# samiwilf/torchrec-oldfork

Hardware: AMD Instinct MI355X
Metric: samples/sec Criteo-1TB DLRM batch 65536 (higher is better)
Workload: dtype f32; 1 GPU; DLRM Criteo-1TB shape: 26 tables (177.9M rows, 84.85 GiB fp32, D=128), 13 dense, pooling factor 1, dense 512-256-128, over 1024-1024-512-256-1, fused exact SGD; global_batch=65536, local_batch=65536, parallelism=mp1: 26 table-wise + 0 row-wise + 0 replicated (data-parallel) tables, dense dp1, ids=uniform, distinct_batches=32, seed=0, data_ranks=1

## Files before the change

include/tbe_hip.h:

```cpp
#ifndef TBE_HIP_H_
#define TBE_HIP_H_

#include <stddef.h>
#include <stdint.h>

#ifdef __cplusplus
extern "C" {
#endif

#define TBE_OK 0
#define TBE_ERR_INVALID_ARGUMENT (-1)
#define TBE_ERR_LAUNCH (-2)
#define TBE_ERR_WORKSPACE (-3)
#define TBE_ERR_UNSUPPORTED (-4)

#define TBE_POOL_SUM 0
#define TBE_POOL_MEAN 1
#define TBE_POOL_NONE 2

#define TBE_OPT_EXACT_SGD 0
#define TBE_OPT_EXACT_ROWWISE_ADAGRAD 1
#define TBE_OPT_ADAM 2
#define TBE_OPT_EXACT_ADAGRAD 3
#define TBE_OPT_DENSE_GRAD 100
// ... 120 lines not shown
int tbe_block_bucketize(const void* lengths, int32_t len_elem_size, int64_t lengths_size,
                        const void* indices, int32_t idx_elem_size, int64_t N,
                        const void* block_sizes, int32_t F, int32_t my_size,
                        const float* weights, int32_t bucketize_pos, int32_t sequence,
                        void* new_lengths, void* new_indices, float* new_weights,
                        void* new_pos, void* unbucketize_permute, void* workspace,
                        size_t workspace_bytes, void* stream);

int tbe_a2a_pooled_unpack(const float* recv, float* out, const int32_t* dim_sum_per_rank,
                          int32_t W, int32_t B_local, int32_t D_total,
                          int32_t dims_multiple_of_4, float scale, void* stream);
int tbe_a2a_pooled_pack(const float* grad, float* send, const int32_t* dim_sum_per_rank,
                        int32_t W, int32_t B_local, int32_t D_total,
                        int32_t dims_multiple_of_4, float scale, void* stream);

int tbe_pooled_exchange_unpack(const float* recv, float* out, const int32_t* feat_out_col,
                               const int32_t* feat_src, const int32_t* feat_slab_col,
                               const int64_t* slab_offset, const int32_t* slab_stride,
                               int32_t Fg, int32_t W, int32_t B_local, int32_t D_total,
                               int32_t all_multiple_of_4, float scale, void* stream);
int tbe_pooled_exchange_pack(const float* grad, float* send, const int32_t* feat_out_col,
                             const int32_t* feat_src, const int32_t* feat_slab_col,
                             const int64_t* slab_offset, const int32_t* slab_stride,
                             int32_t Fg, int32_t W, int32_t B_local, int32_t D_total,
                             int32_t all_multiple_of_4, float scale, void* stream);

int tbe_dlrm_interaction_forward_f32(const float* dense, const float* sparse, int32_t B,
                                     int32_t F, int32_t D, float* out, int64_t out_row_stride,
                                     void* stream);
int tbe_dlrm_interaction_backward_f32(const float* dense, const float* sparse,
                                      const float* grad_out, int64_t grad_row_stride, int32_t B, int32_t F, int32_t D,
                                      float* grad_dense, float* grad_sparse, void* stream);

size_t tbe_relu_backward_bias_grad_workspace_bytes(int64_t B, int32_t N);
int tbe_relu_backward_bias_grad_f32(const float* grad_out, const float* act, int64_t B, int32_t N,
                                    float* grad_in, float* bias_grad, void* workspace,
                                    size_t workspace_bytes, void* stream);

size_t tbe_weighted_colsum_workspace_bytes(int64_t B, int32_t N);
int tbe_weighted_colsum_f32(const float* x, const float* w, int64_t B, int32_t N, float* out,
                            void* workspace, size_t workspace_bytes, void* stream);

int64_t tbe_colsum_row_blocks(int64_t B, int32_t N);
int tbe_relu_backward_bias_partials_f32(const float* grad_out, const float* act, int64_t B, int32_t N,
                                        float* grad_in, float* partial, size_t partial_bytes, void* stream);
int tbe_weighted_colsum_partials_f32(const float* x, const float* w, int64_t B, int32_t N, float* partial,
                                     size_t partial_bytes, void* stream);

int tbe_multi_chunk_sum_f32(const int64_t* seg_table, int32_t nseg, int64_t max_numel, float* dst, float scale,
                            void* stream);
int tbe_multi_chunk_sum_host_table_f32(const int64_t* host_seg_table, int32_t nseg, int64_t max_numel, float* dst,
                                       float scale, void* stream);

size_t tbe_bce_with_logits_workspace_bytes(void);
int tbe_bce_with_logits_f32(const float* logits, const void* labels, int32_t label_elem_size, int64_t B, float* loss,
                            float* dlogits, void* workspace, size_t workspace_bytes, void* stream);

int tbe_jagged_2d_to_dense_f32(const float* values, const int64_t* offsets, int32_t B,
                               int32_t D, int32_t max_L, float* dense, void* stream);

int tbe_dense_to_jagged_2d_f32(const float* dense, const int64_t* offsets, int32_t B, int32_t D,
                               int32_t max_L, int64_t N, float* values, void* stream);

int tbe_offsets_range(const int64_t* offsets, int64_t n, int64_t range_size, int64_t* out,
                      void* stream);

// ... 8 lines not shown
```

torchrec-oldfork_amd/csrc/dlrm_interaction.hip:

```cpp
#include <algorithm>
#include <cstdlib>

#include "common.hpp"

namespace tbe {

using f32x4 = __attribute__((ext_vector_type(4))) float;

__device__ __forceinline__ void wave_lds_fence() { __builtin_amdgcn_wave_barrier(); }

__device__ __forceinline__ int triu_index(int i, int j, int R) { return i * (2 * R - i - 1) / 2 + (j - i - 1); }

__device__ __forceinline__ int triu_row(int p, int R) {
  const int t = 2 * R - 1;
  int i = static_cast<int>((static_cast<float>(t) - sqrtf(static_cast<float>(t * t - 8 * p))) * 0.5f);
  i = max(0, min(i, R - 2));
  while (i + 1 <= R - 2 && (i + 1) * (2 * R - (i + 1) - 1) / 2 <= p) ++i;
  while (i > 0 && i * (2 * R - i - 1) / 2 > p) --i;
  return i;
}

template <int D>
struct XLoader {
  static constexpr int LOG_V = (D == 16 ? 2 : D == 32 ? 3 : D == 64 ? 4 : D == 128 ? 5 : 6);
// ... 365 lines not shown
    wave_lds_fence();
#pragma unroll
    for (int m = 0; m < 2; ++m)
#pragma unroll
      for (int n = 0; n < NT; ++n)
#pragma unroll
        for (int q = 0; q < 4; ++q) {
          const int row = 16 * m + 4 * kq + q;
          if (row < R) xs[row * XS + 16 * n + r16] = acc[m][n][q];
        }
    wave_lds_fence();
#pragma unroll
    for (int i = 0; i < MAXV; ++i) {
      const int v = lane + i * kWave;
      if (v < nvec) {
        const int r = v >> LOG_V;
        const int c = (v & ((1 << LOG_V) - 1)) * 4;
        float4 x = ld4(xs + r * XS + c);
        if (r == 0) {
          x.x += gdense.x;
          x.y += gdense.y;
          x.z += gdense.z;
          x.w += gdense.w;
          st4(grad_dense + static_cast<int64_t>(b) * D + c, x);
        } else {
          st4(grad_sparse + (static_cast<int64_t>(b) * F + (r - 1)) * D + c, x);
        }
      }
    }
    wave_lds_fence();
  }
}

}

using namespace tbe;

static unsigned interaction_grid(int B) {
  const int64_t want = (static_cast<int64_t>(B) + 3) / 4;
  return static_cast<unsigned>(std::max<int64_t>(1, std::min<int64_t>(want, 256 * 2)));
}

template <typename K>
static bool reserve_lds(K kernel, size_t bytes) {
  return hipFuncSetAttribute(reinterpret_cast<const void*>(kernel), hipFuncAttributeMaxDynamicSharedMemorySize,
                             static_cast<int>(bytes)) == hipSuccess;
}

extern "C" int tbe_dlrm_interaction_forward_f32(const float* dense, const float* sparse, int32_t B, int32_t F,
                                                int32_t D, float* out, int64_t out_row_stride, void* stream) {
  TBE_REQUIRE(B >= 0 && F >= 1 && F <= 31, "tbe_dlrm_interaction_forward_f32: F=%d outside [1, 31]", F);
  TBE_REQUIRE(out_row_stride >= D + (F + 1) * F / 2, "tbe_dlrm_interaction_forward_f32: out_row_stride %lld < D + F(F+1)/2",
              (long long)out_row_stride);
  TBE_REQUIRE(D == 16 || D == 32 || D == 64 || D == 128 || D == 256,
              "tbe_dlrm_interaction_forward_f32: D=%d not in {16,32,64,128,256}", D);
  if (B == 0) return TBE_OK;
  TBE_REQUIRE(dense && sparse && out, "tbe_dlrm_interaction_forward_f32: null pointer");
  TBE_REQUIRE(((reinterpret_cast<uintptr_t>(dense) | reinterpret_cast<uintptr_t>(sparse)) & 15) == 0,
              "tbe_dlrm_interaction_forward_f32: inputs must be 16-B aligned");
  const int R = F + 1, P = R * (R - 1) / 2;
  const size_t lds = 4 * static_cast<size_t>((P + 3) & ~3) * sizeof(float);
  hipStream_t st = static_cast<hipStream_t>(stream);
  const int64_t want = (static_cast<int64_t>(B) + 3) / 4;
  const dim3 grid(static_cast<unsigned>(std::max<int64_t>(1, std::min<int64_t>(want, 256 * (D <= 128 ? 4 : 2)))));
  if (D == 64 || D == 128) {
    const int rpi = 64 / (D / 4);
// ... 33 lines not shown
  TBE_REQUIRE(B >= 0 && F >= 1 && F <= 27, "tbe_dlrm_interaction_backward_f32: F=%d outside [1, 27]", F);
  TBE_REQUIRE(grad_row_stride >= D + (F + 1) * F / 2, "tbe_dlrm_interaction_backward_f32: grad_row_stride %lld < D + F(F+1)/2",
              (long long)grad_row_stride);
  TBE_REQUIRE(D == 16 || D == 32 || D == 64 || D == 128, "tbe_dlrm_interaction_backward_f32: D=%d not in {16,32,64,128}", D);
  if (B == 0) return TBE_OK;
  TBE_REQUIRE(dense && sparse && grad_out && grad_dense && grad_sparse, "tbe_dlrm_interaction_backward_f32: null pointer");
  TBE_REQUIRE(((reinterpret_cast<uintptr_t>(dense) | reinterpret_cast<uintptr_t>(sparse) |
                reinterpret_cast<uintptr_t>(grad_dense) | reinterpret_cast<uintptr_t>(grad_sparse)) & 15) == 0,
              "tbe_dlrm_interaction_backward_f32: tensors must be 16-B aligned");
  hipStream_t st = static_cast<hipStream_t>(stream);
  const size_t lds = 4 * (static_cast<size_t>(28) * (D + 16) + 32 * 34) * sizeof(float);
  const dim3 grid(interaction_grid(B));
  static bool attr_set = false;
  if (!attr_set) {
    const size_t big = 4 * (28 * (128 + 16) + 32 * 34) * sizeof(float);
    if (!reserve_lds(interaction_bwd_kernel<8>, big) || !reserve_lds(interaction_bwd_kernel<4>, big)) {
      set_error("tbe_dlrm_interaction_backward_f32: cannot reserve LDS");
      return TBE_ERR_LAUNCH;
    }
    attr_set = true;
  }
#define TBE_IB(NT) \
  hipLaunchKernelGGL(interaction_bwd_kernel<NT>, grid, dim3(256), lds, st, dense, sparse, grad_out, grad_dense, grad_sparse, B, F, grad_row_stride)
  switch (D) {
    case 16: TBE_IB(1); break;
    case 32: TBE_IB(2); break;
    case 64: TBE_IB(4); break;
    default: TBE_IB(8); break;
  }
#undef TBE_IB
  TBE_CHECK_LAUNCH("tbe_dlrm_interaction_backward_f32");
  return TBE_OK;
}
```

torchrec-oldfork_amd/fbgemm_gpu/_lib.py:

```python
import ctypes
import os
from typing import Optional

import torch

_HERE = os.path.dirname(os.path.abspath(__file__))
LIB_PATH = os.path.normpath(os.path.join(_HERE, "..", "lib", "libtbe_hip.so"))

c_void_p = ctypes.c_void_p
c_i32 = ctypes.c_int32
c_i64 = ctypes.c_int64
c_size = ctypes.c_size_t
c_float = ctypes.c_float


class OptimizerArgs(ctypes.Structure):

    _fields_ = [
        ("optimizer", c_i32),
        ("learning_rate", c_float),
        ("eps", c_float),
        ("weight_decay", c_float),
        ("beta1", c_float),
        ("beta2", c_float),
# ... 67 lines not shown
    "tbe_permute_2d_workspace_bytes": (c_size, [c_i32, c_i32, c_i32]),
    "tbe_permute_2d_lengths": (
        ctypes.c_int,
        [c_void_p, c_i32, c_i32, c_i32, c_void_p, c_i32, c_void_p, c_void_p, c_void_p, c_void_p,
         c_size, c_void_p],
    ),
    "tbe_permute_2d_data": (
        ctypes.c_int,
        [c_void_p, c_i32, c_i32, c_void_p, c_void_p, c_void_p, c_void_p, c_i32, c_void_p, c_void_p,
         c_i32, c_void_p],
    ),
    "tbe_bucketize_workspace_bytes": (c_size, [c_i64, c_i32]),
    "tbe_block_bucketize": (
        ctypes.c_int,
        [c_void_p, c_i32, c_i64, c_void_p, c_i32, c_i64, c_void_p, c_i32, c_i32, c_void_p, c_i32,
         c_i32, c_void_p, c_void_p, c_void_p, c_void_p, c_void_p, c_void_p, c_size, c_void_p],
    ),
    "tbe_a2a_pooled_unpack": (
        ctypes.c_int, [c_void_p, c_void_p, c_void_p, c_i32, c_i32, c_i32, c_i32, c_float, c_void_p]),
    "tbe_a2a_pooled_pack": (
        ctypes.c_int, [c_void_p, c_void_p, c_void_p, c_i32, c_i32, c_i32, c_i32, c_float, c_void_p]),
    "tbe_pooled_exchange_unpack": (
        ctypes.c_int,
        [c_void_p, c_void_p, c_void_p, c_void_p, c_void_p, c_void_p, c_void_p, c_i32, c_i32, c_i32,
         c_i32, c_i32, c_float, c_void_p]),
    "tbe_pooled_exchange_pack": (
        ctypes.c_int,
        [c_void_p, c_void_p, c_void_p, c_void_p, c_void_p, c_void_p, c_void_p, c_i32, c_i32, c_i32,
         c_i32, c_i32, c_float, c_void_p]),
    "tbe_dlrm_interaction_forward_f32": (
        ctypes.c_int, [c_void_p, c_void_p, c_i32, c_i32, c_i32, c_void_p, c_i64, c_void_p]),
    "tbe_dlrm_interaction_backward_f32": (
        ctypes.c_int, [c_void_p, c_void_p, c_void_p, c_i64, c_i32, c_i32, c_i32, c_void_p, c_void_p, c_void_p]),
    "tbe_relu_backward_bias_grad_workspace_bytes": (c_size, [c_i64, c_i32]),
    "tbe_relu_backward_bias_grad_f32": (
        ctypes.c_int, [c_void_p, c_void_p, c_i64, c_i32, c_void_p, c_void_p, c_void_p, c_size, c_void_p]),
    "tbe_weighted_colsum_workspace_bytes": (c_size, [c_i64, c_i32]),
    "tbe_weighted_colsum_f32": (
        ctypes.c_int, [c_void_p, c_void_p, c_i64, c_i32, c_void_p, c_void_p, c_size, c_void_p]),
    "tbe_colsum_row_blocks": (c_i64, [c_i64, c_i32]),
    "tbe_relu_backward_bias_partials_f32": (
        ctypes.c_int, [c_void_p, c_void_p, c_i64, c_i32, c_void_p, c_void_p, c_size, c_void_p]),
    "tbe_weighted_colsum_partials_f32": (
        ctypes.c_int, [c_void_p, c_void_p, c_i64, c_i32, c_void_p, c_size, c_void_p]),
    "tbe_multi_chunk_sum_f32": (ctypes.c_int, [c_void_p, c_i32, c_i64, c_void_p, c_float, c_void_p]),
    "tbe_multi_chunk_sum_host_table_f32": (ctypes.c_int, [c_void_p, c_i32, c_i64, c_void_p, c_float, c_void_p]),
    "tbe_bce_with_logits_workspace_bytes": (c_size, []),
    "tbe_bce_with_logits_f32": (
        ctypes.c_int, [c_void_p, c_void_p, c_i32, c_i64, c_void_p, c_void_p, c_void_p, c_size, c_void_p]),
    "tbe_jagged_2d_to_dense_f32": (
        ctypes.c_int, [c_void_p, c_void_p, c_i32, c_i32, c_i32, c_void_p, c_void_p]),
    "tbe_dense_to_jagged_2d_f32": (
        ctypes.c_int, [c_void_p, c_void_p, c_i32, c_i32, c_i32, c_i64, c_void_p, c_void_p]),
    "tbe_offsets_range": (ctypes.c_int, [c_void_p, c_i64, c_i64, c_void_p, c_void_p]),
    "tbe_copy_rows": (ctypes.c_int, [c_void_p, c_i64, c_void_p, c_i32, c_i64, c_void_p, c_void_p]),
}

_lib: Optional[ctypes.CDLL] = None


def load() -> ctypes.CDLL:
    global _lib
    if _lib is not None:
        return _lib
    if not os.path.exists(LIB_PATH):
        raise ImportError(
# ... 77 lines not shown
```

torchrec-oldfork_amd/fbgemm_gpu/split_table_batched_embeddings_ops.py:

```python
import enum
import os
import types
from ctypes import byref as ctypes_byref
from dataclasses import dataclass
from typing import List, Optional, Tuple

import torch
from torch import nn

from . import _lib, _streams
from ._lib import CacheDesc, OptimizerArgs, check, ptr, raise_on_faults, require_gpu, stream_ptr, workspace
from .split_embedding_configs import EmbOptimType as OptimType
from .split_embedding_configs import SparseType


_FLAG_WEIGHTED = 2


class EmbeddingLocation(enum.IntEnum):
    DEVICE = 0
    MANAGED = 1
    MANAGED_CACHING = 2
    HOST = 3

# ... 878 lines not shown
        prepare = torch.is_grad_enabled() and (
            mode in (True, "1") or (mode == "auto" and indices.numel() <= self.overlap_backward_sort_max_ids))
        out = _FusedLookup.apply(self.placeholder_autograd_tensor, self, indices, offsets,
                                 per_sample_weights, B, prepare)
        self._enforce_bounds_check_mode()
        return out

    def forward_into(self, out: torch.Tensor, out_offsets: torch.Tensor, row_stride: int, indices: torch.Tensor,
                     offsets: torch.Tensor, per_sample_weights: Optional[torch.Tensor] = None) -> torch.Tensor:
        indices, offsets, per_sample_weights, B = self._check_inputs(indices, offsets, per_sample_weights)
        if self._cache is not None:
            indices = self._cache.prefetch(self._real_layout(), indices, offsets, B, torch.is_grad_enabled())
        mode = self.overlap_backward_sort
        prepare = torch.is_grad_enabled() and (
            mode in (True, "1") or (mode == "auto" and indices.numel() <= self.overlap_backward_sort_max_ids))
        out = _FusedLookupInto.apply(out, self.placeholder_autograd_tensor, self, indices, offsets,
                                     per_sample_weights, B, out_offsets, int(row_stride), prepare)
        self._enforce_bounds_check_mode()
        return out

    def lookup_no_autograd(self, indices: torch.Tensor, offsets: torch.Tensor,
                           per_sample_weights: Optional[torch.Tensor] = None, into=None):
        indices, offsets, per_sample_weights, B = self._check_inputs(indices, offsets, per_sample_weights)
        if self._cache is not None:
            indices = self._cache.prefetch(self._real_layout(), indices, offsets, B, True)
        rec = LookupRecord(indices, offsets, per_sample_weights, B, (into[1], int(into[2])) if into is not None else None)
        out = self._forward_impl(indices, offsets, per_sample_weights, B, into=into)
        mode = self.overlap_backward_sort
        if mode in (True, "1") or (mode == "auto" and indices.numel() <= self.overlap_backward_sort_max_ids_explicit):
            rec.prepared = self._prepare_or_defer(rec, indices, offsets, B, per_sample_weights is not None)
        self._enforce_bounds_check_mode()
        return out, rec

    def backward_no_autograd(self, rec: "LookupRecord", grad_out: torch.Tensor) -> None:
        self.iter += 1
        self._backward_impl(grad_out, rec.indices, rec.offsets, rec.per_sample_weights, rec.B, self._optimizer_struct(),
                            prepared=rec.prepared, layout=rec.layout)
        rec.prepared = None
        if self._cache is not None:
            self._cache.after_backward()


class _DenseLookup(torch.autograd.Function):
    @staticmethod
    def forward(ctx, weights, module, indices, offsets, per_sample_weights, B):
        ctx.module = module
        ctx.B = B
        ctx.save_for_backward(indices, offsets, per_sample_weights)
        return module._forward_impl(indices, offsets, per_sample_weights, B)

    @staticmethod
    def backward(ctx, grad_out):
        indices, offsets, psw = ctx.saved_tensors
        module = ctx.module
        grad_w = torch.zeros_like(module.weights)
        state0 = module._dense_grad_ptrs(grad_w)
        opt = OptimizerArgs(_OPT_DENSE_GRAD, 0.0, 0.0, 0.0, 0.0, 0.0, 1)
        module._backward_impl(grad_out, indices, offsets, psw, ctx.B, opt, state0_override=state0,
                              state0_aligned=grad_w.data_ptr() % 16 == 0)
        return grad_w, None, None, None, None, None


class DenseTableBatchedEmbeddingBagsCodegen(_TBEBase):

    def __init__(
        self,
# ... 81 lines not shown
```

torchrec-oldfork_amd/torchrec_amd/distributed/embeddingbag.py:

```python
import os
from typing import Any, Callable, Dict, Iterator, List, Optional, Tuple

import torch
import torch.distributed as dist
from torch import nn

from ..modules.embedding_configs import EmbeddingBagConfig, pooling_type_to_pooling_mode
from ..modules.embedding_modules import EmbeddingBagCollection
from ..profiling import label
from ..sparse.jagged_tensor import KeyedJaggedTensor, KeyedTensor
from . import _device_ops
from .planner import rw_block_size, rw_shard_rows
from .types import Awaitable, LazyAwaitable, NoWait, ParameterSharding, ShardingEnv, ShardingType

GRADIENT_DIVISION = True
FORCE_EXCHANGE = os.environ.get("TORCHREC_AMD_FORCE_EXCHANGE", "0") == "1"


def set_gradient_division(val: bool) -> None:
    global GRADIENT_DIVISION
    GRADIENT_DIVISION = val


def _gather_rows(mat: torch.Tensor, order: List[int], order_dev: torch.Tensor) -> torch.Tensor:
# ... 900 lines not shown
            buf = self._output_buffer
            use_buf = buf is not None and buf.numel() == B * self._D_total
            if self._dp_module is None and not use_buf:
                emb = self._emb_module(dist_input.values, dist_input.offsets, dist_input.weights)
                return NoWait(KeyedTensor(keys, lpe, emb))
            out = (self._alias_output_buffer(B) if use_buf
                   else torch.empty((B, self._D_total), dtype=torch.float32, device=self._device))
            if self._emb_module is not None:
                out = self._emb_module.forward_into(out, self._sharded_out_off, self._D_total, dist_input.values,
                                                    dist_input.offsets, dist_input.weights)
            return NoWait(KeyedTensor(keys, lpe, self._dp_fill(out, dist_input)))
        if self._emb_module is not None:
            with label("## tbe_lookup ##"):
                emb = self._emb_module(dist_input.values, dist_input.offsets, dist_input.weights)
        else:
            emb = torch.zeros((self._world_size * B, 0), dtype=torch.float32, device=self._device,
                              requires_grad=True)
        state = _ExchangeState(self, B)
        recv = _ExchangeReq.apply(emb, state)
        return _OutputAwaitable(
            lambda: KeyedTensor(keys, lpe, self._dp_fill(_ExchangeWait.apply(recv, state), dist_input)))

    def explicit_step_supported(self, batch_size: int) -> bool:
        buf = self._output_buffer
        return (self._emb_module is not None and buf is not None
                and buf.numel() == batch_size * self._D_total and hasattr(self._emb_module, "lookup_no_autograd")
                and (self._dp_module is None or hasattr(self._dp_module, "lookup_no_autograd")))

    def compute_explicit(self, dist_input: SparseFeaturesDist, prefetched: bool = False) -> "ExplicitLookupStep":
        if not self.explicit_step_supported(dist_input.batch_size):
            raise RuntimeError("compute_explicit: not available for this configuration (explicit_step_supported())")
        return ExplicitLookupStep(self, dist_input, halves=self.half_batch_exchange, early_replicated_lookup=not prefetched)

    def forward(self, features: KeyedJaggedTensor) -> Awaitable[KeyedTensor]:
        return self.compute_and_output_dist(self.input_dist(features).wait())


class ExplicitLookupStep:

    def __init__(self, owner: "ShardedEmbeddingBagCollection", dist_input: SparseFeaturesDist, halves: bool = False,
                 early_replicated_lookup: bool = True) -> None:
        self.o, self.d = owner, dist_input
        self.halves = bool(halves and owner._exchange)
        self.epoch = owner._weights_epoch
        self.dp_rec = None
        self.state: Optional[_ExchangeState] = None
        self._grad: Optional[torch.Tensor] = None
        self._early_dp = False
        self._dp_sort_pending = False
        if owner._exchange:
            m = owner._emb_module
            can_defer = hasattr(m, "launch_deferred_backward_sort") and not getattr(m, "defer_backward_sort", False)
            if can_defer:
                m.defer_backward_sort = True
            try:
                with label("## tbe_lookup ##"):
                    emb, self.rec = m.lookup_no_autograd(dist_input.values, dist_input.offsets, dist_input.weights)
            finally:
                if can_defer:
                    m.defer_backward_sort = False
            self.state = _ExchangeState(owner, dist_input.batch_size)
            if self.halves:
                self.state.start_forward_halves(emb)
            else:
                self.state.start_forward(emb, allow_static=True)
            self._early_dp = owner._dp_module is not None and early_replicated_lookup
            if self._early_dp:
                v, offs, w = dist_input.dp
# ... 114 lines not shown
```

torchrec-oldfork_amd/torchrec_amd/distributed/train_pipeline.py:

```python
from typing import Any, Iterator, List, Optional, Tuple

import torch

from fbgemm_gpu._streams import side_stream

from ..profiling import label
from .model_parallel import DistributedModelParallel


class _PipelinedEBC:

    def __init__(self, sharded, pipeline: "TrainPipelineSparseDist") -> None:
        self.sharded = sharded
        self.pipeline = pipeline

    def _dist_input(self, features):
        req = self.pipeline._requests.pop(id(self.sharded), None)
        if req is None:
            return self.sharded.input_dist(features).wait()
        cur = torch.cuda.current_stream()
        with label("## wait_sparse_data_dist ##"):
            with torch.cuda.stream(self.pipeline._data_dist_stream):
                dist_in = req.wait()
            cur.wait_stream(self.pipeline._data_dist_stream)
        dist_in.record_stream(cur)
        return dist_in

    def forward(self, features):
        return self.sharded.compute_and_output_dist(self._dist_input(features))

    def compute_explicit(self, features, prefetched: bool = False):
        if not hasattr(self.sharded, "compute_explicit") or not self.sharded.explicit_step_supported(features.stride()):
            return None
        return self.sharded.compute_explicit(self._dist_input(features), prefetched=prefetched)


class TrainPipelineSparseDist:
    def __init__(self, model: torch.nn.Module, optimizer: Any, device: torch.device, hip_graphs: bool = False,
                 prefetch_lookup: Optional[bool] = None) -> None:
        self._model, self._optimizer, self._device = model, optimizer, device
        self._hip_graphs = hip_graphs and device.type == "cuda"
        if isinstance(model, DistributedModelParallel) and model.is_data_parallel_wrapped():
            self._hip_graphs = False
        use_streams = device.type == "cuda"
        self._memcpy_stream = side_stream(device) if use_streams else None
        self._data_dist_stream = side_stream(device) if use_streams else None
        self._requests = {}
        import os
        env = os.environ.get("TORCHREC_AMD_PREFETCH_LOOKUP")
        self._prefetch = bool(prefetch_lookup) if prefetch_lookup is not None else (env == "1" if env is not None else None)
        self._batch_i = None
        self._batch_ip1 = None
        self._batch_ip2 = None
        self._connected = False
        dmp = model if isinstance(model, DistributedModelParallel) else None
        self._sharded = dmp.sharded_modules() if dmp is not None else []
        self._install()

    def _install(self) -> None:
        self._wrappers: List[_PipelinedEBC] = []
        for s in self._sharded:
            w = getattr(s, "_pipelined", None)
            if w is None or w.pipeline is not self:
                w = _PipelinedEBC(s, self)
                s.forward = w.forward
                s._pipelined = w
            self._wrappers.append(w)
# ... 114 lines not shown
```

torchrec-oldfork_amd/torchrec_amd/models/dlrm.py:

```python
import os
from typing import Dict, List, Optional, Tuple

import torch
from torch import nn

from ..modules.mlp import MLP, LinearOut
from ..profiling import label
from ..sparse.jagged_tensor import KeyedJaggedTensor, KeyedTensor


class SparseArch(nn.Module):

    def __init__(self, embedding_bag_collection: nn.Module) -> None:
        super().__init__()
        self.embedding_bag_collection = embedding_bag_collection
        cfgs = embedding_bag_collection.embedding_bag_configs
        assert cfgs, "Embedding bag collection cannot be empty!"
        self.D: int = cfgs[0].embedding_dim
        self._sparse_feature_names: List[str] = [n for c in cfgs for n in c.feature_names]
        self.F: int = len(self._sparse_feature_names)

    def start(self, features: KeyedJaggedTensor):
        return self.embedding_bag_collection(features)

# ... 61 lines not shown
        buf = torch.empty((B, stride), dtype=torch.float32, device=dense.device)
        with torch.cuda.device(dense.device):
            check(_lib.load().tbe_dlrm_interaction_forward_f32(ptr(dense), ptr(sparse), B, F, D, ptr(buf), stride,
                                                               stream_ptr(dense.device)),
                  "tbe_dlrm_interaction_forward_f32")
        ctx.save_for_backward(dense, sparse)
        ctx.grad_sinks = grad_sinks
        return buf if stride == width else buf[:, :width]

    @staticmethod
    def backward(ctx, grad_out):
        from fbgemm_gpu import _lib
        from fbgemm_gpu._lib import check, ptr, stream_ptr

        dense, sparse = ctx.saved_tensors
        B, F, D = sparse.shape
        width = D + (F + 1) * F // 2
        if grad_out.shape != (B, width):
            raise RuntimeError(f"dot interaction backward: grad_out {tuple(grad_out.shape)} has the wrong shape")
        if grad_out.dtype != torch.float32 or grad_out.stride(1) != 1 or grad_out.stride(0) < width:
            grad_out = grad_out.float().contiguous()
        if ctx.grad_sinks is not None:
            gd, gs = ctx.grad_sinks
            if (gd.shape != dense.shape or gs.shape != sparse.shape or not gd.is_contiguous() or not gs.is_contiguous()
                    or gd.dtype != torch.float32 or gs.dtype != torch.float32 or gd.device != dense.device):
                raise RuntimeError("dot interaction backward: gradient sinks do not match the inputs")
        else:
            gd, gs = torch.empty_like(dense), torch.empty_like(sparse)
        with torch.cuda.device(dense.device):
            check(_lib.load().tbe_dlrm_interaction_backward_f32(ptr(dense), ptr(sparse), ptr(grad_out), grad_out.stride(0),
                                                                B, F, D, ptr(gd), ptr(gs), stream_ptr(dense.device)),
                  "tbe_dlrm_interaction_backward_f32")
        return gd, gs, None, None


def _fused_interaction_ok(dense: torch.Tensor, sparse: torch.Tensor) -> bool:
    F, D = sparse.shape[1], sparse.shape[2]
    return (dense.is_cuda and dense.dtype == torch.float32 and sparse.dtype == torch.float32
            and 1 <= F <= 27 and D in (16, 32, 64, 128))


class InteractionArch(nn.Module):

    def __init__(self, num_sparse_features: int) -> None:
        super().__init__()
        self.F = num_sparse_features
        self.fused = True
        self.pad_rows = os.environ.get("TORCHREC_AMD_PAD_INTERACTION", "0") == "1"
        self.grad_sinks = None
        self.register_buffer("triu_indices", torch.triu_indices(self.F + 1, self.F + 1, offset=1), persistent=False)

    def forward(self, dense_features: torch.Tensor, sparse_features: torch.Tensor) -> torch.Tensor:
        if self.F <= 0:
            return dense_features
        if self.fused and _fused_interaction_ok(dense_features, sparse_features):
            return _FusedDotInteraction.apply(dense_features, sparse_features, self.pad_rows, self.grad_sinks)
        combined = torch.cat((dense_features.unsqueeze(1), sparse_features), dim=1)
        interactions = torch.bmm(combined, combined.transpose(1, 2))
        flat = interactions[:, self.triu_indices[0], self.triu_indices[1]]
        return torch.cat((dense_features, flat), dim=1)


class OverArch(nn.Module):
    def __init__(self, in_features: int, layer_sizes: List[int], device: Optional[torch.device] = None) -> None:
        super().__init__()
        if len(layer_sizes) <= 1:
            raise ValueError("OverArch must have multiple layers.")
        self.model = nn.Sequential(
            MLP(in_features, layer_sizes[:-1], bias=True, activation="relu", device=device),
            LinearOut(layer_sizes[-2], layer_sizes[-1], bias=True, device=device))

    def forward(self, features: torch.Tensor) -> torch.Tensor:
        return self.model(features)


class DLRM(nn.Module):
    def __init__(self, embedding_bag_collection: nn.Module, dense_in_features: int,
                 dense_arch_layer_sizes: List[int], over_arch_layer_sizes: List[int],
                 dense_device: Optional[torch.device] = None) -> None:
        super().__init__()
        cfgs = embedding_bag_collection.embedding_bag_configs
        assert len(cfgs) > 0, "At least one embedding bag is required"
        D = cfgs[0].embedding_dim
        assert all(c.embedding_dim == D for c in cfgs), "All EmbeddingBagConfigs must have the same dimension"
        if dense_arch_layer_sizes[-1] != D:
            raise ValueError(f"embedding_bag_collection dimension ({D}) and final dense arch layer size "
                             f"({dense_arch_layer_sizes[-1]}) must match.")
        self.sparse_arch = SparseArch(embedding_bag_collection)
        F = self.sparse_arch.F
        self.dense_arch = DenseArch(dense_in_features, dense_arch_layer_sizes, device=dense_device)
        self.inter_arch = InteractionArch(F)
        over_in = D + (F + 1) * F // 2
        self.over_arch = OverArch(over_in, over_arch_layer_sizes, device=dense_device)
        if dense_device is not None:
            self.inter_arch.to(dense_device)

    def forward(self, dense_features: torch.Tensor, sparse_features: KeyedJaggedTensor) -> torch.Tensor:
        pending = self.sparse_arch.start(sparse_features)
        embedded_dense = self.dense_arch(dense_features)
        embedded_sparse = self.sparse_arch.finish(pending)
        concatenated = self.inter_arch(dense_features=embedded_dense, sparse_features=embedded_sparse)
        return self.over_arch(concatenated)




class _FusedBCEWithLogits(torch.autograd.Function):
    @staticmethod
    def forward(ctx, logits, labels):
        from ..distributed import _device_ops

        loss, dlogits = torch.ops.tbe_hip.bce_with_logits(logits, labels)
        ctx.save_for_backward(dlogits)
        return loss

    @staticmethod
    def backward(ctx, grad_out):
        (dlogits,) = ctx.saved_tensors
        return dlogits * grad_out, None


def bce_with_logits_mean(loss_fn: nn.Module, logits: torch.Tensor, labels: torch.Tensor) -> torch.Tensor:
    if (logits.is_cuda and logits.dtype == torch.float32 and logits.dim() == 1 and labels.shape == logits.shape
            and type(loss_fn) is nn.BCEWithLogitsLoss and loss_fn.reduction == "mean" and loss_fn.weight is None
            and loss_fn.pos_weight is None and logits.numel() > 0 and labels.dtype in (torch.float32, torch.int64)):
        return _FusedBCEWithLogits.apply(logits, labels)
    return loss_fn(logits, labels.float())


class _Head(nn.Module):
# ... 455 lines not shown
```

Measured before the change: 7.747 million samples/s.

## Fuse embedding row gather into DLRM interaction forward and backward kernels

Adds gather-interaction kernels that read embedding rows straight from the table weights by index (pooling factor 1), so the separate TBE pooled-output write and re-read is skipped. The forward uses LDS-DMA loads with software prefetch of the next sample's ids and rows. The backward re-gathers the rows to compute gradients and then calls the fused SGD backward directly. A deferred lookup path in the sharded EBC and DLRM forward turns this on when single-rank, table-wise, fixed-length-1 conditions hold. The cost is extra random row reads in backward and new code paths that only cover restricted configurations.

```diff
diff --git a/include/tbe_hip.h b/include/tbe_hip.h
--- a/include/tbe_hip.h
+++ b/include/tbe_hip.h
@@ -176,6 +176,15 @@
                                       const float* grad_out, int64_t grad_row_stride, int32_t B, int32_t F, int32_t D,
                                       float* grad_dense, float* grad_sparse, void* stream);
 
+int tbe_dlrm_interaction_gather_forward_f32(const float* dense, const uint64_t* feat_weights, const int64_t* feat_rows,
+                                            const int64_t* feat_window, const int64_t* indices, int32_t B, int32_t F,
+                                            int32_t D, float* out, int64_t out_row_stride, int32_t* bounds_errors,
+                                            void* stream);
+int tbe_dlrm_interaction_gather_backward_f32(const float* dense, const uint64_t* feat_weights, const int64_t* feat_rows,
+                                             const int64_t* feat_window, const int64_t* indices, const float* grad_out,
+                                             int64_t grad_row_stride, int32_t B, int32_t F, int32_t D, float* grad_dense,
+                                             float* grad_sparse, int32_t* bounds_errors, void* stream);
+
 size_t tbe_relu_backward_bias_grad_workspace_bytes(int64_t B, int32_t N);
 int tbe_relu_backward_bias_grad_f32(const float* grad_out, const float* act, int64_t B, int32_t N,
                                     float* grad_in, float* bias_grad, void* workspace,
diff --git a/torchrec-oldfork_amd/csrc/dlrm_interaction.hip b/torchrec-oldfork_amd/csrc/dlrm_interaction.hip
--- a/torchrec-oldfork_amd/csrc/dlrm_interaction.hip
+++ b/torchrec-oldfork_amd/csrc/dlrm_interaction.hip
@@ -421,6 +421,350 @@
   }
 }
 
+
+__device__ __attribute__((aligned(16))) float g_zero_row[256];
+
+struct GatherLane {
+  RowWindow win;
+  uint64_t base;
+  bool counts;
+};
+__device__ __forceinline__ GatherLane load_gather_lane(const uint64_t* feat_weights, const int64_t* feat_rows,
+                                                       const int64_t* feat_window, int lane, int F) {
+  GatherLane g;
+  const int f = min(lane, F - 1);
+  g.win = load_window(feat_rows, feat_window, f);
+  g.base = feat_weights[f];
+  g.counts = lane < F;
+  return g;
+}
+template <int D>
+__device__ __forceinline__ uint64_t gather_row_address(const GatherLane& g, int64_t id, uint64_t miss, int& nbad) {
+  int64_t local;
+  const int cls = classify_id(g.win, id, local);
+  if (cls == kIdBad && g.counts) ++nbad;
+  return cls == kIdLocal ? g.base + static_cast<uint64_t>(local) * (D * sizeof(float)) : miss;
+}
+__device__ __forceinline__ void report_bad_ids(int nbad, int32_t* bounds_errors) {
+  if (bounds_errors == nullptr) return;
+#pragma unroll
+  for (int o = 32; o > 0; o >>= 1) nbad += __shfl_xor(nbad, o, kWave);
+  if ((threadIdx.x & 63) == 0 && nbad > 0) atomicAdd(bounds_errors, nbad);
+}
+
+template <int D>
+__global__ __launch_bounds__(256, 2) void interaction_gather_fwd_kernel(const float* __restrict__ dense,
+                                                                       const uint64_t* __restrict__ feat_weights,
+                                                                       const int64_t* __restrict__ feat_rows,
+                                                                       const int64_t* __restrict__ feat_window,
+                                                                       const int64_t* __restrict__ indices,
+                                                                       float* __restrict__ out,
+                                                                       int32_t* __restrict__ bounds_errors, int B, int F,
+                                                                       int64_t out_stride) {
+  extern __shared__ float smem[];
+  constexpr int NS = D / 16;
+  constexpr int PR = D / 4;
+  constexpr int RPI = kWave / PR;
+  constexpr int IDS = 64;
+  static_assert(PR >= 16 && PR <= kWave, "LDS-DMA form needs 64 <= D <= 256");
+  const int lane = threadIdx.x & 63;
+  const int wave = threadIdx.x >> 6;
+  const int R = F + 1;
+  const int P = R * (R - 1) / 2;
+  const int P4 = (P + 3) & ~3;
+  const int NI = (R + RPI - 1) / RPI;
+  float* xs = smem + wave * (NI * RPI * D + P4 + IDS);
+  float* zs = xs + NI * RPI * D;
+  float* ids = zs + P4;
+  const bool vec_out = (out_stride & 3) == 0 && out_stride >= D + P4 && (reinterpret_cast<uintptr_t>(out) & 15) == 0;
+  if (lane < P4 - P) zs[P + lane] = 0.f;
+  const int r16 = lane & 15;
+  const int kq = lane >> 4;
+  const int row0 = min(r16, R - 1);
+  const int row1 = min(16 + r16, R - 1);
+  const int stride_b = gridDim.x * 4;
+  const GatherLane gl = load_gather_lane(feat_weights, feat_rows, feat_window, lane, F);
+  const uint64_t zero_row = reinterpret_cast<uint64_t>(&g_zero_row[0]);
+  int nbad = 0;
+  const uint32_t* id_words = reinterpret_cast<const uint32_t*>(indices) +
+                             2 * static_cast<int64_t>(min(lane >> 1, F - 1)) * B + (lane & 1);
+  auto issue_ids = [&](int b) {
+    __builtin_amdgcn_global_load_lds((const __attribute__((address_space(1))) void*)(id_words + 2 * static_cast<int64_t>(b)),
+                                     (__attribute__((address_space(3))) void*)ids, 4, 0, 0);
+  };
+  auto issue_copy = [&](int b, uint64_t row_addr) {
+    const uint64_t dn = reinterpret_cast<uint64_t>(dense + static_cast<int64_t>(b) * D);
+#pragma unroll 1
+    for (int i = 0; i < NI; ++i) {
+      const int row = min(i * RPI + lane / PR, R - 1);
+      const int piece = (lane % PR) ^ (row & 15);
+      uint64_t src = shflu64(row_addr, max(row - 1, 0));
+      if (row == 0) src = dn;
+      src += 16 * piece;
+      __builtin_amdgcn_global_load_lds((const __attribute__((address_space(1))) void*)src,
+                                       (__attribute__((address_space(3))) void*)(xs + i * (kWave * 4)), 16, 0, 0);
+    }
+  };
+  auto read_id = [&]() { return *reinterpret_cast<const int64_t*>(ids + 2 * min(lane, F - 1)); };
+  const bool dense_lane = lane < PR;
+  const int T = (P + kWave - 1) / kWave;
+  constexpr int DS = (D + kWave - 1) / kWave;
+  int stores_behind_copy = 0;
+  int b = blockIdx.x * 4 + wave;
+  if (b < B) {
+    issue_ids(b);
+    vm_wait_all_but<0>();
+    __builtin_amdgcn_wave_barrier();
+    const int64_t id = read_id();
+    asm volatile("s_waitcnt lgkmcnt(0)" ::: "memory");
+    __builtin_amdgcn_wave_barrier();
+    issue_copy(b, gather_row_address<D>(gl, id, zero_row, nbad));
+    if (b + stride_b < B) issue_ids(b + stride_b);
+  }
+  for (; b < B; b += stride_b) {
+    vm_wait_all_but(stores_behind_copy);
+    __builtin_amdgcn_wave_barrier();
+    float4 xa[NS], xb[NS];
+#pragma unroll
+    for (int s = 0; s < NS; ++s) xa[s] = *reinterpret_cast<const float4*>(xs + row0 * D + 4 * ((4 * s + kq) ^ (row0 & 15)));
+    if (R > 16) {
+#pragma unroll
+      for (int s = 0; s < NS; ++s) xb[s] = *reinterpret_cast<const float4*>(xs + row1 * D + 4 * ((4 * s + kq) ^ (row1 & 15)));
+    } else {
+#pragma unroll
+      for (int s = 0; s < NS; ++s) xb[s] = make_float4(0.f, 0.f, 0.f, 0.f);
+    }
+    float4 dpass = make_float4(0.f, 0.f, 0.f, 0.f);
+    float dscal[DS];
+    if (vec_out) {
+      if (dense_lane) dpass = *reinterpret_cast<const float4*>(xs + 4 * lane);
+    } else {
+#pragma unroll
+      for (int t = 0; t < DS; ++t) dscal[t] = xs[min(lane + t * kWave, D - 1)];
+    }
+    const int64_t next_id = read_id();
+    asm volatile("s_waitcnt lgkmcnt(0)" ::: "memory");
+    __builtin_amdgcn_wave_barrier();
+    if (b + stride_b < B) {
+      issue_copy(b + stride_b, gather_row_address<D>(gl, next_id, zero_row, nbad));
+      if (b + 2 * stride_b < B) issue_ids(b + 2 * stride_b);
+    }
+    f32x4 acc00 = {0.f, 0.f, 0.f, 0.f}, acc01 = acc00, acc11 = acc00;
+#pragma unroll
+    for (int s = 0; s < NS; ++s) {
+      const float a0[4] = {xa[s].x, xa[s].y, xa[s].z, xa[s].w};
+      const float a1[4] = {xb[s].x, xb[s].y, xb[s].z, xb[s].w};
+#pragma unroll
+      for (int e = 0; e < 4; ++e) {
+        acc00 = __builtin_amdgcn_mfma_f32_16x16x4f32(a0[e], a0[e], acc00, 0, 0, 0);
+        acc01 = __builtin_amdgcn_mfma_f32_16x16x4f32(a0[e], a1[e], acc01, 0, 0, 0);
+        acc11 = __builtin_amdgcn_mfma_f32_16x16x4f32(a1[e], a1[e], acc11, 0, 0, 0);
+      }
+    }
+    float* orow = out + static_cast<int64_t>(b) * out_stride;
+    if (vec_out) {
+      if (dense_lane) st4(orow + lane * 4, dpass);
+    } else {
+#pragma unroll
+      for (int t = 0; t < DS; ++t) vm_store_dword(orow + min(lane + t * kWave, D - 1), dscal[t]);
+    }
+#pragma unroll
+    for (int q = 0; q < 4; ++q) {
+      const int i = kq * 4 + q;
+      const int j = r16;
+      if (i < j && j < R) zs[triu_index(i, j, R)] = acc00[q];
+      if (16 + j < R && i < R) zs[triu_index(i, 16 + j, R)] = acc01[q];
+      if (i < j && 16 + j < R) zs[triu_index(16 + i, 16 + j, R)] = acc11[q];
+    }
+    __builtin_amdgcn_wave_barrier();
+    constexpr int MAXT = 8;
+    constexpr int MAXQ = 2;
+    if (vec_out) {
+#pragma unroll
+      for (int t = 0; t < MAXQ; ++t) {
+        const int q = lane + t * kWave;
+        if (q < P4 / 4) st4(orow + D + 4 * q, *reinterpret_cast<const float4*>(zs + 4 * q));
+      }
+      stores_behind_copy = 0;
+    } else {
+      float zv[MAXT];
+#pragma unroll
+      for (int t = 0; t < MAXT; ++t)
+        if (t < T) zv[t] = zs[min(lane + t * kWave, P - 1)];
+#pragma unroll
+      for (int t = 0; t < MAXT; ++t)
+        if (t < T) vm_store_dword(orow + D + min(lane + t * kWave, P - 1), zv[t]);
+      stores_behind_copy = DS + T;
+    }
+    __builtin_amdgcn_wave_barrier();
+  }
+  report_bad_ids(nbad, bounds_errors);
+}
+
+template <int NT>
+__global__ __launch_bounds__(256, 2) void interaction_gather_bwd_kernel(const float* __restrict__ dense,
+                                                                       const uint64_t* __restrict__ feat_weights,
+                                                                       const int64_t* __restrict__ feat_rows,
+                                                                       const int64_t* __restrict__ feat_window,
+                                                                       const int64_t* __restrict__ indices,
+                                                                       const float* __restrict__ grad_out,
+                                                                       float* __restrict__ grad_dense,
+                                                                       float* __restrict__ grad_sparse,
+                                                                       int32_t* __restrict__ bounds_errors, int B, int F,
+                                                                       int64_t grad_stride) {
+  extern __shared__ float smem[];
+  constexpr int D = NT * 16;
+  constexpr int XS = D + 16;
+  constexpr int GS = 34;
+  constexpr int XROWS = 28;
+  constexpr int LOG_V = XLoader<D>::LOG_V;
+  constexpr int MAXV = (XROWS * D / 4 + kWave - 1) / kWave;
+  const int lane = threadIdx.x & 63;
+  const int wave = threadIdx.x >> 6;
+  const int R = F + 1;
+  const int P = R * (R - 1) / 2;
+  float* xs = smem + wave * (XROWS * XS + 32 * GS);
+  float* gs = xs + XROWS * XS;
+  const int r16 = lane & 15;
+  const int kq = lane >> 4;
+  const int nvec = R * (D / 4);
+  const int ksteps = (R + 3) / 4;
+  const int stride_b = gridDim.x * 4;
+  for (int e = lane; e < XROWS * XS; e += kWave) xs[e] = 0.f;
+  for (int e = lane; e < 32 * GS; e += kWave) gs[e] = 0.f;
+  constexpr int MAXP = (28 * 27 / 2 + kWave - 1) / kWave;
+  int pij[MAXP];
+#pragma unroll
+  for (int t = 0; t < MAXP; ++t) {
+    const int p = lane + t * kWave;
+    int i = 0, j = 1;
+    if (p < P) {
+      i = triu_row(p, R);
+      j = i + 1 + (p - i * (2 * R - i - 1) / 2);
+    }
+    pij[t] = (i << 8) | j;
+  }
+  wave_lds_fence();
+
+  const GatherLane gl = load_gather_lane(feat_weights, feat_rows, feat_window, lane, F);
+  const int64_t* my_ids = indices + static_cast<int64_t>(min(lane, F - 1)) * B;
+  int nbad = 0;
+  float4 pre[MAXV];
+  float gpre[MAXP];
+  auto load_x = [&](int s, uint64_t row_addr) {
+#pragma unroll
+    for (int i = 0; i < MAXV; ++i) {
+      const int v = lane + i * kWave;
+      const int r = min(v >> LOG_V, R - 1);
+      const int c = (v & ((1 << LOG_V) - 1)) * 4;
+      const uint64_t src = shflu64(row_addr, max(r - 1, 0));
+      if (v < nvec) {
+        if (r == 0)
+          pre[i] = ld4(dense + static_cast<int64_t>(s) * D + c);
+        else
+          pre[i] = src != 0 ? ld4(reinterpret_cast<const float*>(src) + c) : make_float4(0.f, 0.f, 0.f, 0.f);
+      }
+    }
+  };
+  int b = blockIdx.x * 4 + wave;
+  int64_t next_id = 0;
+  if (b < B) {
+    load_x(b, gather_row_address<D>(gl, my_ids[b], 0, nbad));
+    if (b + stride_b < B) next_id = my_ids[b + stride_b];
+#pragma unroll
+    for (int t = 0; t < MAXP; ++t) {
+      const int p = lane + t * kWave;
+      gpre[t] = p < P ? grad_out[static_cast<int64_t>(b) * grad_stride + D + p] : 0.f;
+    }
+  }
+  for (; b < B; b += stride_b) {
+#pragma unroll
+    for (int i = 0; i < MAXV; ++i) {
+      const int v = lane + i * kWave;
+      if (v < nvec) st4(xs + (v >> LOG_V) * XS + (v & ((1 << LOG_V) - 1)) * 4, pre[i]);
+    }
+#pragma unroll
+    for (int t = 0; t < MAXP; ++t) {
+      if (lane + t * kWave < P) {
+        const int i = pij[t] >> 8, j = pij[t] & 255;
+        gs[i * GS + j] = gpre[t];
+        gs[j * GS + i] = gpre[t];
+      }
+    }
+    const float* grow = grad_out + static_cast<int64_t>(b) * grad_stride;
+    float4 gdense = make_float4(0.f, 0.f, 0.f, 0.f);
+    if (lane < D / 4) {
+      if (((grad_stride & 3) | (reinterpret_cast<uintptr_t>(grad_out) & 15)) == 0) {
+        gdense = ld4(grow + lane * 4);
+      } else {
+        gdense.x = grow[lane * 4 + 0];
+        gdense.y = grow[lane * 4 + 1];
+        gdense.z = grow[lane * 4 + 2];
+        gdense.w = grow[lane * 4 + 3];
+      }
+    }
+    const int nb = b + stride_b;
+    if (nb < B) {
+      load_x(nb, gather_row_address<D>(gl, next_id, 0, nbad));
+      if (nb + stride_b < B) next_id = my_ids[nb + stride_b];
+#pragma unroll
+      for (int t = 0; t < MAXP; ++t) {
+        const int p = lane + t * kWave;
+        gpre[t] = p < P ? grad_out[static_cast<int64_t>(nb) * grad_stride + D + p] : 0.f;
+      }
+    }
+    wave_lds_fence();
+    f32x4 acc[2][NT];
+#pragma unroll
+    for (int m = 0; m < 2; ++m)
+#pragma unroll
+      for (int n = 0; n < NT; ++n) acc[m][n] = f32x4{0.f, 0.f, 0.f, 0.f};
+    for (int ks = 0; ks < ksteps; ++ks) {
+      const int k = ks * 4 + kq;
+      const float a0 = gs[r16 * GS + k];
+      const float a1 = gs[(16 + r16) * GS + k];
+      const float* xrow = xs + k * XS + r16;
+#pragma unroll
+      for (int n = 0; n < NT; ++n) {
+        const float bn = xrow[16 * n];
+        acc[0][n] = __builtin_amdgcn_mfma_f32_16x16x4f32(a0, bn, acc[0][n], 0, 0, 0);
+        acc[1][n] = __builtin_amdgcn_mfma_f32_16x16x4f32(a1, bn, acc[1][n], 0, 0, 0);
+      }
+    }
+    wave_lds_fence();
+#pragma unroll
+    for (int m = 0; m < 2; ++m)
+#pragma unroll
+      for (int n = 0; n < NT; ++n)
+#pragma unroll
+        for (int q = 0; q < 4; ++q) {
+          const int row = 16 * m + 4 * kq + q;
+          if (row < R) xs[row * XS + 16 * n + r16] = acc[m][n][q];
+        }
+    wave_lds_fence();
+#pragma unroll
+    for (int i = 0; i < MAXV; ++i) {
+      const int v = lane + i * kWave;
+      if (v < nvec) {
+        const int r = v >> LOG_V;
+        const int c = (v & ((1 << LOG_V) - 1)) * 4;
+        float4 x = ld4(xs + r * XS + c);
+        if (r == 0) {
+          x.x += gdense.x;
+          x.y += gdense.y;
+          x.z += gdense.z;
+          x.w += gdense.w;
+          st4(grad_dense + static_cast<int64_t>(b) * D + c, x);
+        } else {
+          st4(grad_sparse + (static_cast<int64_t>(b) * F + (r - 1)) * D + c, x);
+        }
+      }
+    }
+    wave_lds_fence();
+  }
+  report_bad_ids(nbad, bounds_errors);
+}
+
 }
 
 using namespace tbe;
@@ -520,3 +864,81 @@
   TBE_CHECK_LAUNCH("tbe_dlrm_interaction_backward_f32");
   return TBE_OK;
 }
+
+static int check_gather_args(const char* what, int32_t B, int32_t F, int32_t D, int64_t row_stride) {
+  TBE_REQUIRE(B >= 0 && F >= 1 && F <= 27, "%s: F=%d outside [1, 27]", what, F);
+  TBE_REQUIRE(D == 64 || D == 128, "%s: D=%d not in {64,128}", what, D);
+  TBE_REQUIRE(row_stride >= D + (F + 1) * F / 2, "%s: row stride %lld < D + F(F+1)/2", what, (long long)row_stride);
+  return TBE_OK;
+}
+
+extern "C" int tbe_dlrm_interaction_gather_forward_f32(const float* dense, const uint64_t* feat_weights,
+                                                       const int64_t* feat_rows, const int64_t* feat_window,
+                                                       const int64_t* indices, int32_t B, int32_t F, int32_t D, float* out,
+                                                       int64_t out_row_stride, int32_t* bounds_errors, void* stream) {
+  const char* what = "tbe_dlrm_interaction_gather_forward_f32";
+  if (int rc = check_gather_args(what, B, F, D, out_row_stride)) return rc;
+  TBE_REQUIRE(dense && feat_weights && feat_rows && indices && out, "%s: null pointer", what);
+  TBE_REQUIRE((reinterpret_cast<uintptr_t>(dense) & 15) == 0 && (reinterpret_cast<uintptr_t>(indices) & 7) == 0,
+              "%s: dense must be 16-B aligned, indices 8-B aligned", what);
+  if (B == 0) return TBE_OK;
+  const int R = F + 1, P = R * (R - 1) / 2;
+  const int rpi = 64 / (D / 4);
+  const int rows = (R + rpi - 1) / rpi * rpi;
+  const size_t lds = 4 * (static_cast<size_t>(rows) * D + ((P + 3) & ~3) + 64) * sizeof(float);
+  static bool attr_set = false;
+  if (!attr_set) {
+    const size_t big = 4 * (static_cast<size_t>(28) * 128 + 380 + 64) * sizeof(float);
+    if (!reserve_lds(interaction_gather_fwd_kernel<128>, big) || !reserve_lds(interaction_gather_fwd_kernel<64>, big)) {
+      set_error("%s: cannot reserve LDS", what);
+      return TBE_ERR_LAUNCH;
+    }
+    attr_set = true;
+  }
+  hipStream_t st = static_cast<hipStream_t>(stream);
+  const dim3 grid(interaction_grid(B));
+  if (D == 128)
+    hipLaunchKernelGGL(interaction_gather_fwd_kernel<128>, grid, dim3(256), lds, st, dense, feat_weights, feat_rows,
+                       feat_window, indices, out, bounds_errors, B, F, out_row_stride);
+  else
+    hipLaunchKernelGGL(interaction_gather_fwd_kernel<64>, grid, dim3(256), lds, st, dense, feat_weights, feat_rows,
+                       feat_window, indices, out, bounds_errors, B, F, out_row_stride);
+  TBE_CHECK_LAUNCH(what);
+  return TBE_OK;
+}
+
+extern "C" int tbe_dlrm_interaction_gather_backward_f32(const float* dense, const uint64_t* feat_weights,
+                                                        const int64_t* feat_rows, const int64_t* feat_window,
+                                                        const int64_t* indices, const float* grad_out,
+                                                        int64_t grad_row_stride, int32_t B, int32_t F, int32_t D,
+                                                        float* grad_dense, float* grad_sparse, int32_t* bounds_errors,
+                                                        void* stream) {
+  const char* what = "tbe_dlrm_interaction_gather_backward_f32";
+  if (int rc = check_gather_args(what, B, F, D, grad_row_stride)) return rc;
+  TBE_REQUIRE(dense && feat_weights && feat_rows && indices && grad_out && grad_dense && grad_sparse, "%s: null pointer",
+              what);
+  TBE_REQUIRE(((reinterpret_cast<uintptr_t>(dense) | reinterpret_cast<uintptr_t>(grad_dense) |
+                reinterpret_cast<uintptr_t>(grad_sparse)) & 15) == 0 && (reinterpret_cast<uintptr_t>(indices) & 7) == 0,
+              "%s: tensors must be 16-B aligned, indices 8-B aligned", what);
+  if (B == 0) return TBE_OK;
+  hipStream_t st = static_cast<hipStream_t>(stream);
+  const size_t lds = 4 * (static_cast<size_t>(28) * (D + 16) + 32 * 34) * sizeof(float);
+  static bool attr_set = false;
+  if (!attr_set) {
+    const size_t big = 4 * (28 * (128 + 16) + 32 * 34) * sizeof(float);
+    if (!reserve_lds(interaction_gather_bwd_kernel<8>, big) || !reserve_lds(interaction_gather_bwd_kernel<4>, big)) {
+      set_error("%s: cannot reserve LDS", what);
+      return TBE_ERR_LAUNCH;
+    }
+    attr_set = true;
+  }
+  const dim3 grid(interaction_grid(B));
+  if (D == 128)
+    hipLaunchKernelGGL(interaction_gather_bwd_kernel<8>, grid, dim3(256), lds, st, dense, feat_weights, feat_rows,
+                       feat_window, indices, grad_out, grad_dense, grad_sparse, bounds_errors, B, F, grad_row_stride);
+  else
+    hipLaunchKernelGGL(interaction_gather_bwd_kernel<4>, grid, dim3(256), lds, st, dense, feat_weights, feat_rows,
+                       feat_window, indices, grad_out, grad_dense, grad_sparse, bounds_errors, B, F, grad_row_stride);
+  TBE_CHECK_LAUNCH(what);
+  return TBE_OK;
+}
diff --git a/torchrec-oldfork_amd/fbgemm_gpu/_lib.py b/torchrec-oldfork_amd/fbgemm_gpu/_lib.py
--- a/torchrec-oldfork_amd/fbgemm_gpu/_lib.py
+++ b/torchrec-oldfork_amd/fbgemm_gpu/_lib.py
@@ -123,6 +123,13 @@
         ctypes.c_int, [c_void_p, c_void_p, c_i32, c_i32, c_i32, c_void_p, c_i64, c_void_p]),
     "tbe_dlrm_interaction_backward_f32": (
         ctypes.c_int, [c_void_p, c_void_p, c_void_p, c_i64, c_i32, c_i32, c_i32, c_void_p, c_void_p, c_void_p]),
+    "tbe_dlrm_interaction_gather_forward_f32": (
+        ctypes.c_int,
+        [c_void_p, c_void_p, c_void_p, c_void_p, c_void_p, c_i32, c_i32, c_i32, c_void_p, c_i64, c_void_p, c_void_p]),
+    "tbe_dlrm_interaction_gather_backward_f32": (
+        ctypes.c_int,
+        [c_void_p, c_void_p, c_void_p, c_void_p, c_void_p, c_void_p, c_i64, c_i32, c_i32, c_i32, c_void_p, c_void_p,
+         c_void_p, c_void_p]),
     "tbe_relu_backward_bias_grad_workspace_bytes": (c_size, [c_i64, c_i32]),
     "tbe_relu_backward_bias_grad_f32": (
         ctypes.c_int, [c_void_p, c_void_p, c_i64, c_i32, c_void_p, c_void_p, c_void_p, c_size, c_void_p]),
diff --git a/torchrec-oldfork_amd/fbgemm_gpu/split_table_batched_embeddings_ops.py b/torchrec-oldfork_amd/fbgemm_gpu/split_table_batched_embeddings_ops.py
--- a/torchrec-oldfork_amd/fbgemm_gpu/split_table_batched_embeddings_ops.py
+++ b/torchrec-oldfork_amd/fbgemm_gpu/split_table_batched_embeddings_ops.py
@@ -934,6 +934,27 @@
         self._enforce_bounds_check_mode()
         return out, rec
 
+    def gather_layout(self):
+        if (self._cache is not None or self.pooling_mode != PoolingMode.SUM or self._feature_pooling is not None
+                or any(p != "dev" for p in self.placement) or len(set(self.dims_per_table)) != 1 or self.max_D % 4 != 0
+                or self.bounds_check_mode == BoundsCheckMode.FATAL or self.current_device.type != "cuda"
+                or self.weights_dev.dtype != torch.float32 or self.weights_dev.data_ptr() % 16 != 0):
+            return None
+        lay = self._get_layout()
+        return lay.feat_weights, lay.feat_rows, lay.feat_window
+
+    def lookup_deferred(self, indices: torch.Tensor, offsets: torch.Tensor) -> "LookupRecord":
+        if self._cache is not None:
+            raise RuntimeError("lookup_deferred: not available with MANAGED_CACHING tables (the cache rewrites the ids)")
+        indices, offsets, _, B = self._check_inputs(indices, offsets, None)
+        rec = LookupRecord(indices, offsets, None, B, None)
+        mode = self.overlap_backward_sort
+        if torch.is_grad_enabled() and (
+                mode in (True, "1") or (mode == "auto" and indices.numel() <= self.overlap_backward_sort_max_ids)):
+            rec.prepared = self._prepare_or_defer(rec, indices, offsets, B, False)
+        self._enforce_bounds_check_mode()
+        return rec
+
     def backward_no_autograd(self, rec: "LookupRecord", grad_out: torch.Tensor) -> None:
         self.iter += 1
         self._backward_impl(grad_out, rec.indices, rec.offsets, rec.per_sample_weights, rec.B, self._optimizer_struct(),
diff --git a/torchrec-oldfork_amd/torchrec_amd/distributed/embeddingbag.py b/torchrec-oldfork_amd/torchrec_amd/distributed/embeddingbag.py
--- a/torchrec-oldfork_amd/torchrec_amd/distributed/embeddingbag.py
+++ b/torchrec-oldfork_amd/torchrec_amd/distributed/embeddingbag.py
@@ -956,8 +956,38 @@
             raise RuntimeError("compute_explicit: not available for this configuration (explicit_step_supported())")
         return ExplicitLookupStep(self, dist_input, halves=self.half_batch_exchange, early_replicated_lookup=not prefetched)
 
+    def deferred_lookup_supported(self, features: KeyedJaggedTensor) -> bool:
+        m = self._emb_module
+        if (self._exchange or self._world_size != 1 or self._dp_module is not None or m is None
+                or not hasattr(m, "lookup_deferred") or self._is_weighted
+                or self._local_feats[self._rank] != list(range(len(self._feature_names)))):
+            return False
+        fixed = features.fixed_lengths()
+        F = len(self._feature_names)
+        if (fixed is None or len(fixed) != F or any(n != 1 for n in fixed)
+                or features.values().numel() != F * features.stride() or features.weights_or_none() is not None):
+            return False
+        return m.gather_layout() is not None
+
+    def compute_deferred(self, dist_input: SparseFeaturesDist) -> "DeferredLookup":
+        m = self._emb_module
+        with label("## tbe_lookup ##"):
+            rec = m.lookup_deferred(dist_input.values, dist_input.offsets)
+        return DeferredLookup(m, rec, len(self._feature_names), self._lengths_per_embedding[0])
+
     def forward(self, features: KeyedJaggedTensor) -> Awaitable[KeyedTensor]:
         return self.compute_and_output_dist(self.input_dist(features).wait())
+
+
+class DeferredLookup:
+
+    def __init__(self, module: nn.Module, rec: Any, F: int, D: int) -> None:
+        self.module, self.rec, self.F, self.D, self.B = module, rec, F, D, rec.B
+        self.feat_weights, self.feat_rows, self.feat_window = module.gather_layout()
+
+    def backward(self, grad_sparse: torch.Tensor) -> None:
+        with label("## tbe_backward_fused_optimizer ##"):
+            self.module.backward_no_autograd(self.rec, grad_sparse)
 
 
 class ExplicitLookupStep:
diff --git a/torchrec-oldfork_amd/torchrec_amd/distributed/train_pipeline.py b/torchrec-oldfork_amd/torchrec_amd/distributed/train_pipeline.py
--- a/torchrec-oldfork_amd/torchrec_amd/distributed/train_pipeline.py
+++ b/torchrec-oldfork_amd/torchrec_amd/distributed/train_pipeline.py
@@ -33,6 +33,12 @@
         if not hasattr(self.sharded, "compute_explicit") or not self.sharded.explicit_step_supported(features.stride()):
             return None
         return self.sharded.compute_explicit(self._dist_input(features), prefetched=prefetched)
+
+
+    def compute_deferred(self, features):
+        if not hasattr(self.sharded, "compute_deferred") or not self.sharded.deferred_lookup_supported(features):
+            return None
+        return self.sharded.compute_deferred(self._dist_input(features))
 
 
 class TrainPipelineSparseDist:
diff --git a/torchrec-oldfork_amd/torchrec_amd/models/dlrm.py b/torchrec-oldfork_amd/torchrec_amd/models/dlrm.py
--- a/torchrec-oldfork_amd/torchrec_amd/models/dlrm.py
+++ b/torchrec-oldfork_amd/torchrec_amd/models/dlrm.py
@@ -117,6 +117,55 @@
                                                                 B, F, D, ptr(gd), ptr(gs), stream_ptr(dense.device)),
                   "tbe_dlrm_interaction_backward_f32")
         return gd, gs, None, None
+
+
+class _FusedGatherInteraction(torch.autograd.Function):
+
+    @staticmethod
+    def forward(ctx, dense, placeholder, lookup, pad_rows=False):
+        from fbgemm_gpu import _lib
+        from fbgemm_gpu._lib import check, ptr, stream_ptr
+
+        dense = dense.contiguous()
+        B, F, D = lookup.B, lookup.F, lookup.D
+        if dense.shape != (B, D) or dense.dtype != torch.float32 or dense.device != lookup.module.current_device:
+            raise RuntimeError(f"dot interaction: dense {tuple(dense.shape)} {dense.dtype} on {dense.device} does not match "
+                               f"the lookup (batch {B}, dim {D}, float32 on {lookup.module.current_device})")
+        width = D + (F + 1) * F // 2
+        stride = (D + ((F + 1) * F // 2 + 3) // 4 * 4) if pad_rows else width
+        buf = torch.empty((B, stride), dtype=torch.float32, device=dense.device)
+        with torch.cuda.device(dense.device):
+            check(_lib.load().tbe_dlrm_interaction_gather_forward_f32(
+                ptr(dense), ptr(lookup.feat_weights), ptr(lookup.feat_rows), ptr(lookup.feat_window),
+                ptr(lookup.rec.indices), B, F, D, ptr(buf), stride, lookup.module._errors_ptr(), stream_ptr(dense.device)),
+                "tbe_dlrm_interaction_gather_forward_f32")
+        ctx.save_for_backward(dense)
+        ctx.lookup = lookup
+        return buf if stride == width else buf[:, :width]
+
+    @staticmethod
+    def backward(ctx, grad_out):
+        from fbgemm_gpu import _lib
+        from fbgemm_gpu._lib import check, ptr, stream_ptr
+
+        (dense,) = ctx.saved_tensors
+        lookup, ctx.lookup = ctx.lookup, None
+        B, F, D = lookup.B, lookup.F, lookup.D
+        width = D + (F + 1) * F // 2
+        if grad_out.shape != (B, width):
+            raise RuntimeError(f"dot interaction backward: grad_out {tuple(grad_out.shape)} has the wrong shape")
+        if grad_out.dtype != torch.float32 or grad_out.stride(1) != 1 or grad_out.stride(0) < width:
+            grad_out = grad_out.float().contiguous()
+        gd = torch.empty_like(dense)
+        gs = torch.empty((B, F * D), dtype=torch.float32, device=dense.device)
+        with torch.cuda.device(dense.device):
+            check(_lib.load().tbe_dlrm_interaction_gather_backward_f32(
+                ptr(dense), ptr(lookup.feat_weights), ptr(lookup.feat_rows), ptr(lookup.feat_window),
+                ptr(lookup.rec.indices), ptr(grad_out), grad_out.stride(0), B, F, D, ptr(gd), ptr(gs), None,
+                stream_ptr(dense.device)),
+                "tbe_dlrm_interaction_gather_backward_f32")
+        lookup.backward(gs)
+        return gd, None, None, None
 
 
 def _fused_interaction_ok(dense: torch.Tensor, sparse: torch.Tensor) -> bool:
@@ -179,8 +228,32 @@
         self.over_arch = OverArch(over_in, over_arch_layer_sizes, device=dense_device)
         if dense_device is not None:
             self.inter_arch.to(dense_device)
+        self.fused_lookup = True
+        self.fused_lookup_steps = 0
+
+    def _deferred_lookup(self, dense_features: torch.Tensor, sparse_features: KeyedJaggedTensor):
+        sa = self.sparse_arch
+        ebc = sa.embedding_bag_collection
+        if not (self.fused_lookup and self.inter_arch.fused and 1 <= sa.F <= 27 and sa.D in (64, 128)
+                and dense_features.is_cuda and dense_features.dtype == torch.float32
+                and hasattr(ebc, "deferred_lookup_supported")
+                and list(getattr(ebc, "_feature_names", ())) == list(sa.sparse_feature_names)):
+            return None
+        piped = getattr(ebc, "_pipelined", None)
+        if piped is not None:
+            return piped.compute_deferred(sparse_features)
+        if not ebc.deferred_lookup_supported(sparse_features):
+            return None
+        return ebc.compute_deferred(ebc.input_dist(sparse_features).wait())
 
     def forward(self, dense_features: torch.Tensor, sparse_features: KeyedJaggedTensor) -> torch.Tensor:
+        lookup = self._deferred_lookup(dense_features, sparse_features)
+        if lookup is not None:
+            embedded_dense = self.dense_arch(dense_features)
+            concatenated = _FusedGatherInteraction.apply(embedded_dense, lookup.module.placeholder_autograd_tensor, lookup,
+                                                         self.inter_arch.pad_rows)
+            self.fused_lookup_steps += 1
+            return self.over_arch(concatenated)
         pending = self.sparse_arch.start(sparse_features)
         embedded_dense = self.dense_arch(dense_features)
         embedded_sparse = self.sparse_arch.finish(pending)
```

Measured after the change: 7.991 million samples/s (median of 6 runs). +3.2%, better.
